# csxmli2016/MARCONet

Measured on AMD Instinct MI355X. Metric: SR images/sec (32x512 LR -> 128x2048 SR), higher is better.
Workload: dtype f16x2; 1 GPU; metric config: batch 256 x 32x512 LR, 16 glyphs/img, enc+TSPGAN+TSPSRNet, fp16x2; per_gpu_batch=256, global_batch=256, glyphs_per_image=16, parallelism=dp1, precision_mode=fp16x2, need_prior_image=True, prior_image_precision=fp16, weights=synthetic:tame, collective=none

## Files before the change

### marconet_amd/csrc/upfold_kernels.hip

```cpp
#include "common.h"
#include "../../include/marconet_hip_upfold.h"

#ifndef MNET_UPF_RUN
#define MNET_UPF_RUN 8
#endif

template <typename T>
__global__ void __launch_bounds__(256, 2) upfold_kernel(const T* __restrict__ z, T* __restrict__ y, int H, int W, int C,
                                                        const float* __restrict__ out_scale, const float* __restrict__ bias,
                                                        const float* __restrict__ post_scale, int act, unsigned items_per_image) {
    constexpr int N = Vec<T>::N;
    constexpr int R = MNET_UPF_RUN;
    const unsigned cpp = (unsigned)C / N;
    unsigned bx = blockIdx.x, by = blockIdx.y;
    {
        const unsigned NWG = gridDim.x * gridDim.y, L = by * gridDim.x + bx;
        if ((NWG & 7u) == 0u) { const unsigned V = (L & 7u) * (NWG >> 3) + (L >> 3); by = V / gridDim.x; bx = V - by * gridDim.x; }
    }
    const int n = (int)by;
    const size_t zpix = (size_t)9 * C;
    const T* zbase = z + (size_t)n * H * W * zpix;
    T* ybase = y + (size_t)n * 4 * H * W * C;
    const int W2 = 2 * W;
    for (unsigned id = bx * 256u + threadIdx.x; id < items_per_image; id += gridDim.x * 256u) {
        const unsigned ch = id % cpp, col = id / cpp;
        const int X = (int)(col % (unsigned)W2), y0 = (int)(col / (unsigned)W2) * R, y1 = min(y0 + R, H);
        unsigned c0[3], c1[3];
        float w0[3], w1[3];
#pragma unroll
        for (int kx = 0; kx < 3; ++kx) {
            const int xu = X + kx - 1, xc = min(max(xu, 0), W2 - 1), m = xc >> 1;
            const bool odd = xc & 1, in = xu >= 0 && xu < W2;
            c0[kx] = (unsigned)(odd ? m : max(m - 1, 0)) * (unsigned)zpix;
            c1[kx] = (unsigned)(odd ? min(m + 1, W - 1) : m) * (unsigned)zpix;
            w0[kx] = in ? (odd ? 0.75f : 0.25f) : 0.f;
            w1[kx] = in ? (odd ? 0.25f : 0.75f) : 0.f;
        }
        const T* base = zbase + (size_t)ch * N;
        auto hrow = [&](int r, float (&h)[3][N]) __attribute__((always_inline)) {
            const T* rp = base + (size_t)r * W * zpix;
#pragma unroll
            for (int ky = 0; ky < 3; ++ky) {
#pragma unroll
                for (int kx = 0; kx < 3; ++kx) {
                    const T* tp = rp + (size_t)(3 * ky + kx) * C;
                    float a[N], b[N];
                    unpackr<T>(ldraw<T>(tp + c0[kx]), a);
                    unpackr<T>(ldraw<T>(tp + c1[kx]), b);
#pragma unroll
                    for (int j = 0; j < N; ++j) {
                        const float t = w0[kx] * a[j] + w1[kx] * b[j];
                        h[ky][j] = kx == 0 ? t : h[ky][j] + t;
                    }
                }
                __builtin_amdgcn_sched_barrier(0);
            }
        };
        const float* osp = out_scale ? out_scale + (size_t)n * C + (size_t)ch * N : nullptr;
        const float* bsp = bias ? bias + (size_t)ch * N : nullptr;
        const float* psp = post_scale ? post_scale + (size_t)n * C + (size_t)ch * N : nullptr;
        auto emit1 = [&](T* q, float (&v)[N]) __attribute__((always_inline)) {
            float o[N];
#pragma unroll
            for (int j = 0; j < N; ++j) o[j] = v[j];
            if (osp) {
#pragma unroll
                for (int j = 0; j < N; j += 4) { const f32x4 s4 = *reinterpret_cast<const f32x4*>(osp + j); o[j] *= s4[0]; o[j + 1] *= s4[1]; o[j + 2] *= s4[2]; o[j + 3] *= s4[3]; }
            }
            if (bsp) {
#pragma unroll
                for (int j = 0; j < N; j += 4) { const f32x4 b4 = *reinterpret_cast<const f32x4*>(bsp + j); o[j] += b4[0]; o[j + 1] += b4[1]; o[j + 2] += b4[2]; o[j + 3] += b4[3]; }
            }
            act_apply_vec<N, true>(o, act);
            if (psp) {
#pragma unroll
                for (int j = 0; j < N; j += 4) { const f32x4 p4 = *reinterpret_cast<const f32x4*>(psp + j); o[j] *= p4[0]; o[j + 1] *= p4[1]; o[j + 2] *= p4[2]; o[j + 3] *= p4[3]; }
            }
            straw<T>(q, packr<T>(o));
        };
        float h[3][N];
        float e[N], o[N];
        float ne[N], no[N];
        hrow(max(y0 - 1, 0), h);
        {
            const bool in = y0 > 0;
#pragma unroll
            for (int j = 0; j < N; ++j) {
                e[j] = (in ? 0.75f * h[0][j] : 0.f) + 0.25f * h[1][j];
                o[j] = 0.25f * h[0][j];
            }
        }
        auto centre = [&](int r) __attribute__((always_inline)) {
            const bool up = r > 0, dn = r + 1 < H;
#pragma unroll
            for (int j = 0; j < N; ++j) {
                e[j] += ((up ? 0.25f * h[0][j] : 0.f) + 0.75f * h[1][j]) + 0.75f * h[2][j];
                o[j] += (0.75f * h[0][j] + 0.75f * h[1][j]) + (dn ? 0.25f * h[2][j] : 0.f);
                ne[j] = 0.75f * h[0][j] + 0.25f * h[1][j];
                no[j] = 0.25f * h[0][j];
            }
        };
        hrow(y0, h);
        centre(y0);
        const size_t orow = (size_t)W2 * C;
#pragma unroll 1
        for (int i = y0; i < y1; ++i) {
            hrow(min(i + 1, H - 1), h);
            const bool in = i + 1 < H;
#pragma unroll
            for (int j = 0; j < N; ++j) {
                e[j] += 0.25f * h[2][j];
                o[j] += 0.25f * h[1][j] + (in ? 0.75f * h[2][j] : 0.f);
            }
            T* q = ybase + ((size_t)(2 * i) * W2 + X) * C + (size_t)ch * N;
            emit1(q, e);
            emit1(q + orow, o);
            if (i + 1 < y1) {
#pragma unroll
                for (int j = 0; j < N; ++j) { e[j] = ne[j]; o[j] = no[j]; }
                centre(i + 1);
            }
        }
    }
}

extern "C" int mnet_upfold3x3_nhwc(const void* z, void* y, int32_t dtype, int32_t n, int32_t h, int32_t w, int32_t c,
                                   const float* out_scale, const float* bias, int32_t act, const float* post_scale, void* stream) {
    MNET_CHECK_ARG(z && y && z != y, "upfold3x3: null pointer (or y == z: not an in-place kernel)");
    MNET_CHECK_ARG(n > 0 && n <= 65535 && h > 0 && w > 0 && c > 0, "upfold3x3: bad geometry");
    MNET_CHECK_ARG(is_storage(dtype), "upfold3x3: bad dtype");
    MNET_CHECK_ARG(act == MNET_ACT_NONE || act == MNET_ACT_LRELU || act == MNET_ACT_LRELU_SQRT2, "upfold3x3: activation must be NONE, LRELU or LRELU_SQRT2");
    const int N = chunk_n(dtype);
    MNET_CHECK_ALIGN(c % N == 0 && aligned16(z) && aligned16(y) && aligned16(out_scale) && aligned16(bias) && aligned16(post_scale),
                     "upfold3x3: c %% %d != 0 or unaligned", N);
    MNET_CHECK_ALIGN(!is_split4(dtype) || (c % 32 == 0 && aligned128(z) && aligned128(y)), "upfold3x3: blocked storages need c %% 32 == 0, 128-byte aligned");
    MNET_CHECK_ARG((long long)h * w * (c / N) * 4 < (1ll << 31) && (long long)w * 9 * c < (1ll << 29), "upfold3x3: image too large");
    const long long per = (long long)((h + MNET_UPF_RUN - 1) / MNET_UPF_RUN) * 2 * w * (c / N);
    const int gx = (int)((per + 255) / 256 < 2048 ? (per + 255) / 256 : 2048);
    hipStream_t st = reinterpret_cast<hipStream_t>(stream);
    dispatch_storage(dtype, [&](auto tag) {
        using T = typename decltype(tag)::type;
        hipLaunchKernelGGL((upfold_kernel<T>), dim3(gx, n), dim3(256), 0, st, (const T*)z, (T*)y, h, w, c, out_scale, bias, post_scale, act, (unsigned)per);
    });
    MNET_LAUNCH_CHECK("upfold3x3");
    return MNET_OK;
}
```

Baseline: 273.3 images/s.

## Compute both output column parities per thread in upfold to share loads

Each thread now produces the even and odd output columns for one source column m. It loads the three neighbouring source columns once and uses them for both parities, instead of loading two taps per kx for each output column separately. This roughly halves the thread count and cuts redundant global loads. It also adds byte-offset chunk placement for the split4 storage types and register pinning to steer scheduling. The cost is higher register pressure from doubled accumulators under launch_bounds(256,2).

```diff
diff --git a/marconet_amd/csrc/upfold_cols.h b/marconet_amd/csrc/upfold_cols.h
--- /dev/null
+++ b/marconet_amd/csrc/upfold_cols.h
@@ -0,0 +1,43 @@
+#pragma once
+
+#if defined(__HIPCC__)
+#define UPF_HD __host__ __device__
+#else
+#define UPF_HD
+#endif
+
+enum { UPF_LEFT = 0, UPF_OWN = 1, UPF_RIGHT = 2 };
+
+struct UpfoldTap { int c0, c1, q0, q1; };
+struct UpfoldPairTap { int s0, s1, q0, q1; };
+
+UPF_HD inline int upf_min(int a, int b) { return a < b ? a : b; }
+UPF_HD inline int upf_max(int a, int b) { return a > b ? a : b; }
+
+UPF_HD inline UpfoldTap upfold_tap(int X, int w, int kx) {
+    const int xu = X + kx - 1, xc = upf_min(upf_max(xu, 0), 2 * w - 1), m = xc >> 1;
+    const bool odd = xc & 1, in = xu >= 0 && xu < 2 * w;
+    UpfoldTap t;
+    t.c0 = odd ? m : upf_max(m - 1, 0);
+    t.c1 = odd ? upf_min(m + 1, w - 1) : m;
+    t.q0 = in ? (odd ? 3 : 1) : 0;
+    t.q1 = in ? (odd ? 1 : 3) : 0;
+    return t;
+}
+
+UPF_HD inline int upfold_slot_col(int m, int w, int slot) { return slot == UPF_LEFT ? upf_max(m - 1, 0) : slot == UPF_OWN ? m : upf_min(m + 1, w - 1); }
+
+UPF_HD constexpr bool upfold_pair_loads(int kx, int slot) { return slot == UPF_OWN || (slot == UPF_LEFT ? kx <= 1 : kx >= 1); }
+
+UPF_HD constexpr int upfold_pair_slot0(int par, int kx) { return par + kx <= 1 ? UPF_LEFT : UPF_OWN; }
+
+UPF_HD inline UpfoldPairTap upfold_pair_tap(int m, int w, int par, int kx) {
+    const int d = par + kx - 1;
+    const bool odd = d & 1, in = (d >= 0 || m > 0) && (d <= 1 || m + 1 < w);
+    UpfoldPairTap t;
+    t.s0 = upfold_pair_slot0(par, kx);
+    t.s1 = t.s0 + 1;
+    t.q0 = in ? (odd ? 3 : 1) : 0;
+    t.q1 = in ? (odd ? 1 : 3) : 0;
+    return t;
+}
diff --git a/marconet_amd/csrc/upfold_kernels.hip b/marconet_amd/csrc/upfold_kernels.hip
--- a/marconet_amd/csrc/upfold_kernels.hip
+++ b/marconet_amd/csrc/upfold_kernels.hip
@@ -1,9 +1,48 @@
 #include "common.h"
+#include "upfold_cols.h"
 #include "../../include/marconet_hip_upfold.h"
 
 #ifndef MNET_UPF_RUN
 #define MNET_UPF_RUN 8
 #endif
+
+template <typename T> struct ChunkPlace {
+    unsigned s, a, b;
+    __device__ __forceinline__ explicit ChunkPlace(unsigned ch) {
+        if constexpr (is_split4_type<T>) {
+            s = ch & 3u;
+            a = (ch >> 2) * 128u + s * 16u;
+            b = __is_same(T, hs) ? a + 64u : (ch >> 2) * 128u + 64u + (s < 3u ? s : 2u) * 16u;
+        } else { s = 0u; a = ch * 16u; b = 0u; }
+    }
+};
+template <typename T> __device__ __forceinline__ Raw<T> ldraw_at(const unsigned char* p, unsigned s, unsigned oa, unsigned ob) {
+    Raw<T> r;
+    if constexpr (__is_same(T, hm)) {
+        r.hi = ldg16s(p + oa);
+#if MNET_HM_SIMPLE_LOAD
+        const unsigned char* blk = p + oa - s * 16u;
+        r.lo8 = *reinterpret_cast<const u32x2*>(blk + 64 + hm_lo_slot((int)s) * 8);
+        r.e8 = blk[96];
+#else
+        const u32x4 q = ldg16s(p + ob);
+        const unsigned a0 = (unsigned)__builtin_amdgcn_update_dpp(0, (int)q[0], 0x44, 0xf, 0xf, true);
+        const unsigned a1 = (unsigned)__builtin_amdgcn_update_dpp(0, (int)q[1], 0x44, 0xf, 0xf, true);
+        const unsigned a2 = (unsigned)__builtin_amdgcn_update_dpp(0, (int)q[2], 0x44, 0xf, 0xf, true);
+        const unsigned a3 = (unsigned)__builtin_amdgcn_update_dpp(0, (int)q[3], 0x44, 0xf, 0xf, true);
+        r.lo8 = s < 2u ? u32x2{a0, a1} : u32x2{a2, a3};
+        r.e8 = __builtin_amdgcn_update_dpp(0, (int)q[0], 0xAA, 0xf, 0xf, true) & 0xff;
+#endif
+    } else if constexpr (__is_same(T, hs)) { r.hi = ldg16s(p + oa); r.lo = ldg16s(p + ob); }
+    else r.v = ldg16s(p + oa);
+    return r;
+}
+
+__device__ __forceinline__ void pin2(float& a, float& b) {
+    f32x2 p = {a, b};
+    asm volatile("" : "+v"(p));
+    a = p[0]; b = p[1];
+}
 
 template <typename T>
 __global__ void __launch_bounds__(256, 2) upfold_kernel(const T* __restrict__ z, T* __restrict__ y, int H, int W, int C,
@@ -24,34 +63,51 @@
     const int W2 = 2 * W;
     for (unsigned id = bx * 256u + threadIdx.x; id < items_per_image; id += gridDim.x * 256u) {
         const unsigned ch = id % cpp, col = id / cpp;
-        const int X = (int)(col % (unsigned)W2), y0 = (int)(col / (unsigned)W2) * R, y1 = min(y0 + R, H);
-        unsigned c0[3], c1[3];
-        float w0[3], w1[3];
-#pragma unroll
-        for (int kx = 0; kx < 3; ++kx) {
-            const int xu = X + kx - 1, xc = min(max(xu, 0), W2 - 1), m = xc >> 1;
-            const bool odd = xc & 1, in = xu >= 0 && xu < W2;
-            c0[kx] = (unsigned)(odd ? m : max(m - 1, 0)) * (unsigned)zpix;
-            c1[kx] = (unsigned)(odd ? min(m + 1, W - 1) : m) * (unsigned)zpix;
-            w0[kx] = in ? (odd ? 0.75f : 0.25f) : 0.f;
-            w1[kx] = in ? (odd ? 0.25f : 0.75f) : 0.f;
+        const int m = (int)(col % (unsigned)W), y0 = (int)(col / (unsigned)W) * R, y1 = min(y0 + R, H);
+        const ChunkPlace<T> place(ch);
+        unsigned oa[3], ob[3];
+#pragma unroll
+        for (int s = 0; s < 3; ++s) {
+            const unsigned cs = (unsigned)upfold_slot_col(m, W, s) * (unsigned)zpix * (unsigned)sizeof(T);
+            oa[s] = cs + place.a;
+            ob[s] = cs + place.b;
         }
-        const T* base = zbase + (size_t)ch * N;
-        auto hrow = [&](int r, float (&h)[3][N]) __attribute__((always_inline)) {
-            const T* rp = base + (size_t)r * W * zpix;
+        float w0[2][3], w1[2][3];
+#pragma unroll
+        for (int par = 0; par < 2; ++par) {
+#pragma unroll
+            for (int kx = 0; kx < 3; ++kx) {
+                const UpfoldPairTap t = upfold_pair_tap(m, W, par, kx);
+                w0[par][kx] = 0.25f * (float)t.q0;
+                w1[par][kx] = 0.25f * (float)t.q1;
+            }
+        }
+        auto hrow = [&](int r, float (&h)[2][3][N]) __attribute__((always_inline)) {
+            const T* rp = zbase + (size_t)r * W * zpix;
 #pragma unroll
             for (int ky = 0; ky < 3; ++ky) {
 #pragma unroll
                 for (int kx = 0; kx < 3; ++kx) {
-                    const T* tp = rp + (size_t)(3 * ky + kx) * C;
-                    float a[N], b[N];
-                    unpackr<T>(ldraw<T>(tp + c0[kx]), a);
-                    unpackr<T>(ldraw<T>(tp + c1[kx]), b);
-#pragma unroll
-                    for (int j = 0; j < N; ++j) {
-                        const float t = w0[kx] * a[j] + w1[kx] * b[j];
-                        h[ky][j] = kx == 0 ? t : h[ky][j] + t;
+                    const unsigned char* tp = reinterpret_cast<const unsigned char*>(rp + (size_t)(3 * ky + kx) * C);
+                    float v[3][N];
+#pragma unroll
+                    for (int s = 0; s < 3; ++s) {
+                        if (upfold_pair_loads(kx, s)) unpackr<T>(ldraw_at<T>(tp, place.s, oa[s], ob[s]), v[s]);
                     }
+#pragma unroll
+                    for (int par = 0; par < 2; ++par) {
+                        const int s0 = upfold_pair_slot0(par, kx), s1 = s0 + 1;
+#pragma unroll
+                        for (int j = 0; j < N; ++j) {
+                            const float t = __builtin_fmaf(w0[par][kx], v[s0][j], w1[par][kx] * v[s1][j]);
+                            h[par][ky][j] = kx == 0 ? t : h[par][ky][j] + t;
+                        }
+                    }
+                }
+#pragma unroll
+                for (int par = 0; par < 2; ++par) {
+#pragma unroll
+                    for (int j = 0; j < N; j += 2) pin2(h[par][ky][j], h[par][ky][j + 1]);
                 }
                 __builtin_amdgcn_sched_barrier(0);
             }
@@ -78,49 +134,64 @@
             }
             straw<T>(q, packr<T>(o));
         };
-        float h[3][N];
-        float e[N], o[N];
-        float ne[N], no[N];
+        float h[2][3][N];
+        float e[2][N], o[2][N];
+        float ne[2][N], no[2][N];
         hrow(max(y0 - 1, 0), h);
         {
             const bool in = y0 > 0;
 #pragma unroll
-            for (int j = 0; j < N; ++j) {
-                e[j] = (in ? 0.75f * h[0][j] : 0.f) + 0.25f * h[1][j];
-                o[j] = 0.25f * h[0][j];
+            for (int par = 0; par < 2; ++par) {
+#pragma unroll
+                for (int j = 0; j < N; ++j) {
+                    e[par][j] = (in ? 0.75f * h[par][0][j] : 0.f) + 0.25f * h[par][1][j];
+                    o[par][j] = 0.25f * h[par][0][j];
+                }
             }
         }
         auto centre = [&](int r) __attribute__((always_inline)) {
             const bool up = r > 0, dn = r + 1 < H;
 #pragma unroll
-            for (int j = 0; j < N; ++j) {
-                e[j] += ((up ? 0.25f * h[0][j] : 0.f) + 0.75f * h[1][j]) + 0.75f * h[2][j];
-                o[j] += (0.75f * h[0][j] + 0.75f * h[1][j]) + (dn ? 0.25f * h[2][j] : 0.f);
-                ne[j] = 0.75f * h[0][j] + 0.25f * h[1][j];
-                no[j] = 0.25f * h[0][j];
+            for (int par = 0; par < 2; ++par) {
+#pragma unroll
+                for (int j = 0; j < N; ++j) {
+                    e[par][j] += ((up ? 0.25f * h[par][0][j] : 0.f) + 0.75f * h[par][1][j]) + 0.75f * h[par][2][j];
+                    o[par][j] += (0.75f * h[par][0][j] + 0.75f * h[par][1][j]) + (dn ? 0.25f * h[par][2][j] : 0.f);
+                    ne[par][j] = 0.75f * h[par][0][j] + 0.25f * h[par][1][j];
+                    no[par][j] = 0.25f * h[par][0][j];
+                }
             }
         };
         hrow(y0, h);
         centre(y0);
         const size_t orow = (size_t)W2 * C;
+        int i = y0;
 #pragma unroll 1
-        for (int i = y0; i < y1; ++i) {
+        do {
             hrow(min(i + 1, H - 1), h);
             const bool in = i + 1 < H;
 #pragma unroll
-            for (int j = 0; j < N; ++j) {
-                e[j] += 0.25f * h[2][j];
-                o[j] += 0.25f * h[1][j] + (in ? 0.75f * h[2][j] : 0.f);
-            }
-            T* q = ybase + ((size_t)(2 * i) * W2 + X) * C + (size_t)ch * N;
-            emit1(q, e);
-            emit1(q + orow, o);
+            for (int par = 0; par < 2; ++par) {
+#pragma unroll
+                for (int j = 0; j < N; ++j) {
+                    e[par][j] += 0.25f * h[par][2][j];
+                    o[par][j] += 0.25f * h[par][1][j] + (in ? 0.75f * h[par][2][j] : 0.f);
+                }
+            }
+            T* q = ybase + ((size_t)(2 * i) * W2 + 2 * m) * C + (size_t)ch * N;
+            emit1(q, e[0]);
+            emit1(q + C, e[1]);
+            emit1(q + orow, o[0]);
+            emit1(q + orow + C, o[1]);
             if (i + 1 < y1) {
 #pragma unroll
-                for (int j = 0; j < N; ++j) { e[j] = ne[j]; o[j] = no[j]; }
+                for (int par = 0; par < 2; ++par) {
+#pragma unroll
+                    for (int j = 0; j < N; ++j) { e[par][j] = ne[par][j]; o[par][j] = no[par][j]; }
+                }
                 centre(i + 1);
             }
-        }
+        } while (++i < y1);
     }
 }
 
@@ -135,7 +206,7 @@
                      "upfold3x3: c %% %d != 0 or unaligned", N);
     MNET_CHECK_ALIGN(!is_split4(dtype) || (c % 32 == 0 && aligned128(z) && aligned128(y)), "upfold3x3: blocked storages need c %% 32 == 0, 128-byte aligned");
     MNET_CHECK_ARG((long long)h * w * (c / N) * 4 < (1ll << 31) && (long long)w * 9 * c < (1ll << 29), "upfold3x3: image too large");
-    const long long per = (long long)((h + MNET_UPF_RUN - 1) / MNET_UPF_RUN) * 2 * w * (c / N);
+    const long long per = (long long)((h + MNET_UPF_RUN - 1) / MNET_UPF_RUN) * w * (c / N);
     const int gx = (int)((per + 255) / 256 < 2048 ? (per + 255) / 256 : 2048);
     hipStream_t st = reinterpret_cast<hipStream_t>(stream);
     dispatch_storage(dtype, [&](auto tag) {
```

New measurement: 275.9 images/s, median of 6. Within noise of the previous version (+1.0%).
